# bellaj09/SGC

Hardware: AMD Instinct MI355X
Metric: propagated edges/sec (K-hop SpMM) + precompute wall-time, Reddit K=2 at 1/2/4/8 GPUs (higher is better)
Workload: dtype f32; 1 GPU; reddit-shape sgc_precompute K=2; nodes=232965, undirected_edges=11606919, nnz=23446803, features=602, hops=2, parallelism=single-gpu

## Files before the change

### include/sgc_amd.h

```cpp
#ifndef SGC_AMD_H
#define SGC_AMD_H

#include <stddef.h>
#include <stdint.h>

#ifdef __cplusplus
extern "C" {
#endif

#define SGC_ABI_VERSION 1

enum {
    SGC_OK = 0,
    SGC_EINVAL = 1,
    SGC_ERANGE = 2,
    SGC_EHIP = 3,
    SGC_ENOMEM = 4,
    SGC_EDEVICE = 5
};

int sgc_abi_version(void);
const char *sgc_last_error(void);

int sgc_set_tuning(const char *key, int64_t value);
// ... 238 lines not shown
                         const float *X, int64_t ldx, float *Y, int64_t ldy, int64_t F,
                         int32_t n_threads);
int sgc_spmm_csr_f32_cpu_ex(const int32_t *row_ptr, const int32_t *col_idx, const float *val,
                            int64_t row_begin, int64_t row_end,
                            const float *X, int64_t ldx, float *Y, int64_t ldy, int64_t F,
                            uint32_t flags, int32_t n_threads);
int64_t sgc_propagate_cpu_workspace(int64_t n_rows, int64_t F, int32_t K);
int sgc_propagate_f32_cpu(const int32_t *row_ptr, const int32_t *col_idx, const float *val,
                          int64_t n_rows, const float *X0, int64_t ldx, float *out,
                          int64_t ldo, int64_t F, int32_t K, void *workspace,
                          int64_t workspace_bytes, int32_t n_threads);

int64_t sgc_plan_sorted_workspace(int64_t n_rows);
int sgc_plan_sorted(const int32_t *row_ptr, int64_t row_begin, int64_t row_end,
                    int32_t threshold, int32_t hub_threshold, int32_t *plan, void *workspace,
                    int64_t workspace_bytes, int64_t *counts_host, void *stream);
int sgc_plan_sorted_ex(const int32_t *row_ptr, int64_t row_begin, int64_t row_end,
                       int32_t threshold, int32_t hub_threshold, int32_t *plan, void *workspace,
                       int64_t workspace_bytes, int64_t *counts_host, void *stream);
int sgc_plan_sorted_ex2(const int32_t *row_ptr, int64_t row_begin, int64_t row_end,
                        int32_t threshold, int32_t hub_threshold, int32_t *plan, void *workspace,
                        int64_t workspace_bytes, int64_t *counts_host, void *stream);

int64_t sgc_colsplit_workspace(int64_t n_rows, int32_t groups);
int sgc_csr_colsplit(const int32_t *row_ptr, const int32_t *col_idx, const float *val,
                     int64_t n_rows, int64_t n_cols, int32_t groups, const int32_t *cuts_host,
                     int32_t *row_ptrs, int32_t *col_out, float *val_out, void *workspace,
                     int64_t workspace_bytes, void *stream);
int sgc_csr_colsplit_ex(const int32_t *row_ptr, const int32_t *col_idx, const float *val,
                        int64_t n_rows, int64_t n_cols, int32_t groups,
                        const int32_t *cuts_host, int32_t whole_rows, int32_t *row_ptrs,
                        int32_t *col_out, float *val_out, void *workspace,
                        int64_t workspace_bytes, void *stream);

int sgc_mgpu_init(int ndev, const int *devices);
int sgc_mgpu_attach(const int32_t *row_ptr, const int32_t *col_idx, const float *val,
                    int64_t n_rows, int64_t nnz, void *stream, int64_t *handle);
int sgc_mgpu_propagate(int64_t handle, const float *X0, int64_t ldx, float *out, int64_t ldo,
                       int64_t F, int32_t K, void *stream);
int sgc_mgpu_detach(int64_t handle);
int sgc_mgpu_finalize(void);

enum { SGC_WARM_PROPAGATE = 1, SGC_WARM_CLASSIFIER = 2, SGC_WARM_LOADERS = 4 };
int sgc_warmup(uint32_t units, void *stream);

#ifdef __cplusplus
}
#endif
#endif
```

### sgc_amd/_lib.py

```python
import ctypes
import os

import torch

_HERE = os.path.dirname(os.path.abspath(__file__))
LIB_PATH = os.environ.get("SGC_AMD_LIB", os.path.join(_HERE, "libsgc_amd.so"))

_i64, _i32, _u32 = ctypes.c_int64, ctypes.c_int32, ctypes.c_uint32
_p, _sz = ctypes.c_void_p, ctypes.c_size_t

SIGNATURES = {
    "sgc_abi_version": (ctypes.c_int, []),
    "sgc_last_error": (ctypes.c_char_p, []),
    "sgc_set_tuning": (ctypes.c_int, [ctypes.c_char_p, _i64]),
    "sgc_get_tuning": (_i64, [ctypes.c_char_p]),
    "sgc_coo_to_csr_workspace": (ctypes.c_int, [_i64, _i64, ctypes.POINTER(_sz)]),
    "sgc_coo_to_csr": (ctypes.c_int, [_p, _p, _p, _i64, _i64, _i64, _p, _p, _p, _p, _sz,
                                      ctypes.POINTER(_u32), _p]),
    "sgc_csr64_to_csr": (ctypes.c_int, [_p, _p, _p, _i64, _i64, _i64, _p, _p, _p,
                                        ctypes.POINTER(_u32), _p]),
    "sgc_augnorm_workspace": (_i64, [_i64]),
    "sgc_augnorm_count": (ctypes.c_int, [_p, _p, _p, _i64, _i64, _p, _p, _p, _i64,
                                         ctypes.POINTER(_i64), ctypes.POINTER(_u32), _p]),
    "sgc_augnorm_fill": (ctypes.c_int, [_p, _p, _p, _i64, _p, _p, _p, _p, _p, _i64,
# ... 47 lines not shown
                                                    _i64, _i32, _i32, _i32]),
    "sgc_launch_list_add_pad_rows": (ctypes.c_int, [_i64, _p, _i64, _p, _i64, _i64, _i64, _i32,
                                                    _i32]),
    "sgc_launch_list_run": (ctypes.c_int, [_i64, _p, _p, _p]),
    "sgc_launch_list_destroy": (ctypes.c_int, [_i64]),
    "sgc_linear_f32": (ctypes.c_int, [_p, _i64, _p, _p, _p, _i64, _i64, _i64, _i64, _p]),
    "sgc_linear_kernel_name": (ctypes.c_char_p, [_i64, _i64, _i64, _i64, _p]),
    "sgc_linear_backward_kernel_name": (ctypes.c_char_p, [_i64, _i64, _i64, _i64, _p]),
    "sgc_cross_entropy_workspace": (_i64, [_i64, _i64]),
    "sgc_cross_entropy_f32": (ctypes.c_int, [_p, _i64, _p, _i64, _i64, _i64, _p, _p, _p, _p, _i64,
                                             _p]),
    "sgc_cross_entropy_backward_f32": (ctypes.c_int, [_p, _i64, _p, _p, _p, _p, _i64, _i64, _i64,
                                                      _p, _i64, _p]),
    "sgc_linear_xent_workspace": (_i64, [_i64, _i64, _i64]),
    "sgc_linear_xent_f32": (ctypes.c_int, [_p, _i64, _p, _p, _p, _i64, _i64, _i64, _p, _p, _p,
                                           _p, _i64, _p, _i64, _p]),
    "sgc_timing_enable": (ctypes.c_int, [ctypes.c_int]),
    "sgc_timing_collect": (ctypes.c_int, [_p, _p, _i64, ctypes.POINTER(_i64)]),
    "sgc_timing_collect_ex": (ctypes.c_int, [_p, _p, _p, _p, _i64, ctypes.POINTER(_i64)]),
    "sgc_coo_to_csr_cpu": (ctypes.c_int, [_p, _p, _p, _i64, _i64, _i64, _p, _p, _p,
                                          ctypes.POINTER(_u32)]),
    "sgc_spmm_csr_f32_cpu": (ctypes.c_int, [_p, _p, _p, _i64, _i64, _p, _i64, _p, _i64, _i64,
                                            _i32]),
    "sgc_spmm_csr_f32_cpu_ex": (ctypes.c_int, [_p, _p, _p, _i64, _i64, _p, _i64, _p, _i64, _i64,
                                               ctypes.c_uint32, _i32]),
    "sgc_propagate_cpu_workspace": (_i64, [_i64, _i64, _i32]),
    "sgc_propagate_f32_cpu": (ctypes.c_int, [_p, _p, _p, _i64, _p, _i64, _p, _i64, _i64, _i32,
                                             _p, _i64, _i32]),
    "sgc_colsplit_workspace": (_i64, [_i64, _i32]),
    "sgc_csr_colsplit": (ctypes.c_int, [_p, _p, _p, _i64, _i64, _i32, _p, _p, _p, _p, _p, _i64,
                                        _p]),
    "sgc_csr_colsplit_ex": (ctypes.c_int, [_p, _p, _p, _i64, _i64, _i32, _p, _i32, _p, _p, _p, _p,
                                           _i64, _p]),
    "sgc_plan_sorted_workspace": (_i64, [_i64]),
    "sgc_plan_sorted": (ctypes.c_int, [_p, _i64, _i64, _i32, _i32, _p, _p, _i64, _p, _p]),
    "sgc_plan_sorted_ex": (ctypes.c_int, [_p, _i64, _i64, _i32, _i32, _p, _p, _i64, _p, _p]),
    "sgc_plan_sorted_ex2": (ctypes.c_int, [_p, _i64, _i64, _i32, _i32, _p, _p, _i64, _p, _p]),
    "sgc_mgpu_init": (ctypes.c_int, [ctypes.c_int, _p]),
    "sgc_mgpu_attach": (ctypes.c_int, [_p, _p, _p, _i64, _i64, _p, ctypes.POINTER(_i64)]),
    "sgc_mgpu_propagate": (ctypes.c_int, [_i64, _p, _i64, _p, _i64, _i64, _i32, _p]),
    "sgc_mgpu_detach": (ctypes.c_int, [_i64]),
    "sgc_mgpu_finalize": (ctypes.c_int, []),
    "sgc_warmup": (ctypes.c_int, [_u32, _p]),
    "sgc_linear_backward_workspace": (_i64, [_i64, _i64, _i64]),
    "sgc_linear_backward_f32": (ctypes.c_int, [_p, _i64, _p, _i64, _i64, _i64, _i64, _p, _p, _p,
                                               _i64, _p]),
    "sgc_linear_x16": (ctypes.c_int, [_p, _i32, _i64, _p, _p, _p, _i64, _i64, _i64, _i64, _p]),
    "sgc_linear_x16_kernel_name": (ctypes.c_char_p, [_i64, _i64, _i64, _i64, _p, _i32]),
    "sgc_linear_backward_x16_workspace": (_i64, [_i64, _i64, _i64]),
    "sgc_linear_backward_x16": (ctypes.c_int, [_p, _i32, _i64, _p, _i64, _i64, _i64, _i64, _p, _p,
                                               _p, _i64, _p]),
    "sgc_linear_backward_x16_kernel_name": (ctypes.c_char_p, [_i64, _i64, _i64, _i64, _p, _i32]),
    "sgc_lbfgs_workspace": (_i64, [_i64, _i32]),
    "sgc_lbfgs_init": (ctypes.c_int, [_p, _i64, _i64, _i32, _p]),
    "sgc_lbfgs_begin_step": (ctypes.c_int, [_p, _p]),
    "sgc_lbfgs_iterate_f32": (ctypes.c_int, [_p, _i32, _p, _p, _p, _p, ctypes.c_double, _i32, _i32,
                                             ctypes.c_double, ctypes.c_double, _p]),
    "sgc_lbfgs_read_status": (ctypes.c_int, [_p, ctypes.POINTER(_i64), _p]),
    "sgc_adam_step_f32": (ctypes.c_int, [_i32, _p, _p, _p, _p, _p, _i64, ctypes.c_double,
                                         ctypes.c_double, ctypes.c_double, ctypes.c_double,
                                         ctypes.c_double, _p]),
    "sgc_train_adam_workspace": (_i64, [_i64, _i64, _i64]),
    "sgc_train_adam_f32": (ctypes.c_int, [_p, _i64, _p, _p, _p, _i64, _i64, _i64, _p, _p, _p, _p,
                                          _i64, _i32, ctypes.c_double, ctypes.c_double,
                                          ctypes.c_double, ctypes.c_double, ctypes.c_double, _p,
                                          _p, _i64, _p]),
# ... 46 lines not shown
```

### sgc_amd/csrc/capi.hip

```cpp
#include <cstdarg>
#include <map>
#include <mutex>
#include <vector>
#include <cstdio>
#include <cstring>

#include "common.h"

namespace sgc {

static thread_local char g_err[512] = "";

void set_error(const char *fmt, ...) {
    va_list ap;
    va_start(ap, fmt);
    vsnprintf(g_err, sizeof(g_err), fmt, ap);
    va_end(ap);
}

int coo_to_csr_workspace(int64_t n_rows, int64_t nnz, size_t *bytes);
int coo_to_csr(const int64_t *rows, const int64_t *cols, const float *vals, int64_t nnz,
               int64_t n_rows, int64_t n_cols, int32_t *row_ptr, int32_t *col_idx,
               float *val_out, void *ws, size_t ws_bytes, uint32_t *status_host,
               hipStream_t stream);
// ... 79 lines not shown
const char *linear_backward_kernel_name(int64_t M, int64_t K, int64_t ldx, int64_t C,
                                        const float *X);
int launch_linear_f32(const float *X, int64_t ldx, const float *W, const float *b, float *Y,
                      int64_t ldy, int64_t M, int64_t K, int64_t C, hipStream_t stream);
const char *linear_x16_kernel_name(int64_t M, int64_t K, int64_t ldx, int64_t C, const void *X,
                                   int32_t x_dtype);
int launch_linear_x16(const void *X, int32_t x_dtype, int64_t ldx, const float *W, const float *b,
                      float *Y, int64_t ldy, int64_t M, int64_t K, int64_t C, hipStream_t stream);
const char *linear_backward_x16_kernel_name(int64_t M, int64_t K, int64_t ldx, int64_t C,
                                            const void *X, int32_t x_dtype);
int64_t linear_backward_x16_workspace_bytes(int64_t M, int64_t K, int64_t C);
int linear_backward_x16(const void *X, int32_t x_dtype, int64_t ldx, const float *dY, int64_t ldd,
                        int64_t M, int64_t K, int64_t C, float *dW, float *db, void *ws,
                        int64_t ws_bytes, hipStream_t s);
int64_t plan_sorted_workspace(int64_t n_rows);
int plan_sorted(const int32_t *row_ptr, int64_t row_begin, int64_t row_end, int32_t threshold,
                int32_t hub_threshold, int32_t *plan, void *workspace, int64_t workspace_bytes,
                int64_t *counts_host, hipStream_t stream);
int plan_sorted_ex(const int32_t *row_ptr, int64_t row_begin, int64_t row_end, int32_t threshold,
                   int32_t hub_threshold, int32_t *plan, void *workspace,
                   int64_t workspace_bytes, int64_t *counts_host, hipStream_t stream);
int plan_sorted_ex2(const int32_t *row_ptr, int64_t row_begin, int64_t row_end, int32_t threshold,
                    int32_t hub_threshold, int32_t *plan, void *workspace,
                    int64_t workspace_bytes, int64_t *counts_host, hipStream_t stream);
int64_t colsplit_workspace(int64_t n_rows, int32_t groups);
int colsplit(const int32_t *row_ptr, const int32_t *col_idx, const float *val, int64_t n_rows,
             int64_t n_cols, int32_t groups, const int32_t *cuts_host, int32_t *row_ptrs,
             int32_t *col_out, float *val_out, void *workspace, int64_t workspace_bytes,
             hipStream_t stream);
int colsplit_ex(const int32_t *row_ptr, const int32_t *col_idx, const float *val, int64_t n_rows,
                int64_t n_cols, int32_t groups, const int32_t *cuts_host, int32_t whole_rows,
                int32_t *row_ptrs, int32_t *col_out, float *val_out, void *workspace,
                int64_t workspace_bytes, hipStream_t stream);
int mgpu_init(int ndev, const int *devices);
int mgpu_finalize();
int mgpu_attach(const int32_t *row_ptr, const int32_t *col_idx, const float *val, int64_t n,
                int64_t nnz, hipStream_t stream, int64_t *handle);
int mgpu_detach(int64_t handle);
int mgpu_propagate(int64_t handle, const float *X, int64_t ldx, float *Y, int64_t ldy, int64_t F,
                   int32_t K, hipStream_t stream);
int64_t lbfgs_workspace(int64_t n, int32_t history_size);
int lbfgs_init(void *state, int64_t bytes, int64_t n, int32_t history_size, hipStream_t s);
int lbfgs_begin_step(void *state, hipStream_t s);
int lbfgs_iterate(void *state, int32_t n_tensors, float *const *params, const float *const *grads,
                  const int64_t *numels, const float *loss, double lr, int32_t max_iter,
                  int32_t max_eval, double tol_grad, double tol_change, hipStream_t s);
int lbfgs_read_status(const void *state, int64_t *out_host, hipStream_t s);
extern int g_adam_kernel, g_adam_kernel_last;
int adam_set_tuning(int64_t value);
int64_t adam_small_max_rows();
int adam_step(int32_t n_tensors, float *const *params, const float *const *grads,
              float *const *exp_avgs, float *const *exp_avg_sqs, const int64_t *numels,
              int64_t step, double lr, double beta1, double beta2, double eps, double weight_decay,
              hipStream_t s);
int64_t train_adam_workspace(int64_t M, int64_t K, int64_t C);
int train_adam(const float *X, int64_t ldx, float *W, float *b, const int64_t *labels, int64_t M,
               int64_t K, int64_t C, float *mW, float *vW, float *mb, float *vb, int64_t step0,
               int32_t epochs, double lr, double beta1, double beta2, double eps,
               double weight_decay, float *loss_trace, void *ws, int64_t ws_bytes, hipStream_t s);
hipError_t warm_adam(hipStream_t);

}

using namespace sgc;

extern "C" {
// ... 694 lines not shown
                    int64_t n_rows, int64_t nnz, void *stream, int64_t *handle) {
    return mgpu_attach(row_ptr, col_idx, val, n_rows, nnz, as_stream(stream), handle);
}

int sgc_mgpu_propagate(int64_t handle, const float *X0, int64_t ldx, float *out, int64_t ldo,
                       int64_t F, int32_t K, void *stream) {
    return mgpu_propagate(handle, X0, ldx, out, ldo, F, K, as_stream(stream));
}

int sgc_mgpu_detach(int64_t handle) { return mgpu_detach(handle); }

int sgc_mgpu_finalize(void) { return mgpu_finalize(); }

int64_t sgc_colsplit_workspace(int64_t n_rows, int32_t groups) {
    return colsplit_workspace(n_rows, groups);
}

int sgc_csr_colsplit(const int32_t *row_ptr, const int32_t *col_idx, const float *val,
                     int64_t n_rows, int64_t n_cols, int32_t groups, const int32_t *cuts_host,
                     int32_t *row_ptrs, int32_t *col_out, float *val_out, void *workspace,
                     int64_t workspace_bytes, void *stream) {
    return colsplit(row_ptr, col_idx, val, n_rows, n_cols, groups, cuts_host, row_ptrs, col_out,
                    val_out, workspace, workspace_bytes, as_stream(stream));
}

int sgc_csr_colsplit_ex(const int32_t *row_ptr, const int32_t *col_idx, const float *val,
                        int64_t n_rows, int64_t n_cols, int32_t groups, const int32_t *cuts_host,
                        int32_t whole_rows, int32_t *row_ptrs, int32_t *col_out, float *val_out,
                        void *workspace, int64_t workspace_bytes, void *stream) {
    return colsplit_ex(row_ptr, col_idx, val, n_rows, n_cols, groups, cuts_host, whole_rows,
                       row_ptrs, col_out, val_out, workspace, workspace_bytes, as_stream(stream));
}

int64_t sgc_plan_sorted_workspace(int64_t n_rows) { return plan_sorted_workspace(n_rows); }

int sgc_plan_sorted(const int32_t *row_ptr, int64_t row_begin, int64_t row_end,
                    int32_t threshold, int32_t hub_threshold, int32_t *plan, void *workspace,
                    int64_t workspace_bytes, int64_t *counts_host, void *stream) {
    return plan_sorted(row_ptr, row_begin, row_end, threshold, hub_threshold, plan, workspace,
                       workspace_bytes, counts_host, as_stream(stream));
}

int sgc_plan_sorted_ex2(const int32_t *row_ptr, int64_t row_begin, int64_t row_end,
                        int32_t threshold, int32_t hub_threshold, int32_t *plan, void *workspace,
                        int64_t workspace_bytes, int64_t *counts_host, void *stream) {
    return plan_sorted_ex2(row_ptr, row_begin, row_end, threshold, hub_threshold, plan, workspace,
                           workspace_bytes, counts_host, as_stream(stream));
}

int sgc_plan_sorted_ex(const int32_t *row_ptr, int64_t row_begin, int64_t row_end,
                       int32_t threshold, int32_t hub_threshold, int32_t *plan, void *workspace,
                       int64_t workspace_bytes, int64_t *counts_host, void *stream) {
    return plan_sorted_ex(row_ptr, row_begin, row_end, threshold, hub_threshold, plan, workspace,
                          workspace_bytes, counts_host, as_stream(stream));
}
```

### sgc_amd/csrc/groups.hip

```cpp
#include "common.h"

#include <algorithm>
#include <cstdlib>

namespace sgc {

namespace {

constexpr int kGroupsMax = 8;
constexpr int kThreads = 256;

struct Cuts {
    int32_t c[kGroupsMax + 1];
};

__device__ __forceinline__ int32_t lower_bound(const int32_t *__restrict__ col, int32_t lo,
                                               int32_t hi, int32_t v) {
    while (lo < hi) {
        const int32_t mid = lo + ((hi - lo) >> 1);
        if (col[mid] < v) lo = mid + 1;
        else hi = mid;
    }
    return lo;
}

__global__ void colsplit_count_kernel(const int32_t *__restrict__ row_ptr,
                                      const int32_t *__restrict__ col, int32_t n, int32_t chunk,
                                      int G, Cuts cuts, int32_t whole_rows,
                                      int32_t *__restrict__ counts,
                                      int32_t *__restrict__ block_sums) {
    __shared__ int32_t s_sum[kGroupsMax];
    if (threadIdx.x < kGroupsMax) s_sum[threadIdx.x] = 0;
    __syncthreads();
    const int32_t r0 = blockIdx.x * chunk, r1 = min(n, r0 + chunk);
    int32_t mine[kGroupsMax] = {0, 0, 0, 0, 0, 0, 0, 0};
    for (int32_t r = r0 + threadIdx.x; r < r1; r += blockDim.x) {
        const int32_t k0 = row_ptr[r], k1 = row_ptr[r + 1];
        const bool whole = k1 - k0 <= whole_rows;
        int32_t lo = k0;
        for (int g = 0; g < G; ++g) {
            const int32_t hi =
                (whole || g + 1 == G) ? k1 : lower_bound(col, lo, k1, cuts.c[g + 1]);
            counts[(int64_t)g * n + r] = hi - lo;
            mine[g] += hi - lo;
            lo = hi;
        }
    }
    for (int g = 0; g < G; ++g)
        if (mine[g]) atomicAdd(&s_sum[g], mine[g]);
    __syncthreads();
    if (threadIdx.x < G) block_sums[threadIdx.x * gridDim.x + blockIdx.x] = s_sum[threadIdx.x];
}

__global__ void colsplit_scan_blocks_kernel(int32_t *__restrict__ block_sums, int nblk, int G) {
    if (threadIdx.x != 0 || blockIdx.x != 0) return;
    int32_t run = 0;
    for (int g = 0; g < G; ++g)
        for (int b = 0; b < nblk; ++b) {
            const int32_t v = block_sums[g * nblk + b];
            block_sums[g * nblk + b] = run;
            run += v;
        }
}

__global__ void colsplit_rowptr_kernel(const int32_t *__restrict__ counts, int32_t n,
                                       int32_t chunk, int G,
                                       const int32_t *__restrict__ block_off,
                                       int32_t *__restrict__ row_ptrs) {
    __shared__ int32_t s[kThreads];
    __shared__ int32_t s_carry;
    const int32_t r0 = blockIdx.x * chunk, r1 = min(n, r0 + chunk);
    for (int g = 0; g < G; ++g) {
        const int32_t *cnt = counts + (int64_t)g * n;
        int32_t *rp = row_ptrs + (int64_t)g * (n + 1);
        if (threadIdx.x == 0) s_carry = block_off[g * gridDim.x + blockIdx.x];
        __syncthreads();
        for (int32_t base = r0; base < r1; base += kThreads) {
            const int32_t r = base + threadIdx.x;
            const int32_t v = r < r1 ? cnt[r] : 0;
            s[threadIdx.x] = v;
            __syncthreads();
            for (int o = 1; o < kThreads; o <<= 1) {
                const int32_t add = threadIdx.x >= o ? s[threadIdx.x - o] : 0;
                __syncthreads();
                s[threadIdx.x] += add;
                __syncthreads();
            }
            const int32_t carry = s_carry;
            if (r < r1) rp[r] = carry + s[threadIdx.x] - v;
            __syncthreads();
            if (threadIdx.x == kThreads - 1) s_carry = carry + s[kThreads - 1];
            __syncthreads();
        }
        if (r1 == n && r0 < r1 && threadIdx.x == 0) rp[n] = s_carry;
        __syncthreads();
    }
}

__global__ void colsplit_fill_kernel(const int32_t *__restrict__ row_ptr,
                                     const int32_t *__restrict__ col,
                                     const float *__restrict__ val, int32_t n, int G, Cuts cuts,
                                     int32_t whole_rows, const int32_t *__restrict__ row_ptrs,
                                     int32_t *__restrict__ col_out, float *__restrict__ val_out) {
    const int lane = threadIdx.x & (kWave - 1);
    const int64_t waves = (int64_t)gridDim.x * (blockDim.x / kWave);
    for (int64_t r = (int64_t)blockIdx.x * (blockDim.x / kWave) + threadIdx.x / kWave; r < n;
         r += waves) {
        const int32_t k0 = row_ptr[r], k1 = row_ptr[r + 1];
        if (k1 - k0 <= whole_rows) {
            const int32_t dst = row_ptrs[r];
            for (int32_t k = k0 + lane; k < k1; k += kWave) {
                col_out[dst + (k - k0)] = col[k];
                val_out[dst + (k - k0)] = val[k];
            }
            continue;
        }
        int32_t lo = k0;
        for (int g = 0; g < G; ++g) {
            const int32_t hi = (g + 1 == G) ? k1 : lower_bound(col, lo, k1, cuts.c[g + 1]);
            const int32_t dst = row_ptrs[(int64_t)g * (n + 1) + r];
            for (int32_t k = lo + lane; k < hi; k += kWave) {
                col_out[dst + (k - lo)] = col[k];
                val_out[dst + (k - lo)] = val[k];
            }
            lo = hi;
        }
    }
}

constexpr size_t kAlign = 256;
size_t up(size_t b) { return (b + kAlign - 1) / kAlign * kAlign; }

int nblocks(int64_t n) { return (int)std::max<int64_t>(1, std::min<int64_t>(1024, (n + 1023) / 1024)); }

}

int64_t colsplit_workspace(int64_t n_rows, int32_t groups) {
    if (n_rows <= 0 || groups <= 0) return (int64_t)kAlign;
    return (int64_t)(up((size_t)groups * n_rows * sizeof(int32_t)) +
                     up((size_t)groups * nblocks(n_rows) * sizeof(int32_t)));
}

int colsplit_ex(const int32_t *row_ptr, const int32_t *col_idx, const float *val, int64_t n_rows,
                int64_t n_cols, int32_t groups, const int32_t *cuts_host, int32_t whole_rows,
                int32_t *row_ptrs, int32_t *col_out, float *val_out, void *workspace,
                int64_t workspace_bytes, hipStream_t stream) {
    SGC_REQUIRE(whole_rows >= 0, SGC_EINVAL, "colsplit: whole_rows must be >= 0");
    SGC_REQUIRE(groups >= 1 && groups <= kGroupsMax, SGC_EINVAL,
                "colsplit: groups must be 1..%d", kGroupsMax);
    SGC_REQUIRE(n_rows >= 0 && n_rows < INT32_MAX && n_cols >= 0 && n_cols < INT32_MAX,
                SGC_ERANGE, "colsplit: bad shape");
    SGC_REQUIRE(row_ptr && row_ptrs && cuts_host && workspace, SGC_EINVAL,
                "colsplit: null pointer");
    SGC_REQUIRE(cuts_host[0] == 0 && cuts_host[groups] == n_cols, SGC_EINVAL,
                "colsplit: cuts must run from 0 to n_cols");
    Cuts cuts{};
    for (int g = 0; g <= groups; ++g) {
        SGC_REQUIRE(g == 0 || cuts_host[g] >= cuts_host[g - 1], SGC_EINVAL,
                    "colsplit: cuts must not decrease");
        cuts.c[g] = cuts_host[g];
    }
    if (n_rows == 0) {
        for (int g = 0; g < groups; ++g)
            SGC_HIP_CHECK(hipMemsetAsync(row_ptrs + g, 0, sizeof(int32_t), stream));
        return SGC_OK;
    }
    SGC_REQUIRE(workspace_bytes >= colsplit_workspace(n_rows, groups), SGC_ENOMEM,
                "colsplit: workspace %lld < %lld bytes", (long long)workspace_bytes,
                (long long)colsplit_workspace(n_rows, groups));
    SGC_REQUIRE(col_out && val_out, SGC_EINVAL, "colsplit: null output");
    const int32_t n = (int32_t)n_rows;
    const int nblk = nblocks(n_rows);
    const int32_t chunk = (int32_t)((n_rows + nblk - 1) / nblk);
    char *w = static_cast<char *>(workspace);
    int32_t *counts = reinterpret_cast<int32_t *>(w);
    w += up((size_t)groups * n_rows * sizeof(int32_t));
    int32_t *block_sums = reinterpret_cast<int32_t *>(w);
    hipLaunchKernelGGL(colsplit_count_kernel, dim3(nblk), dim3(kThreads), 0, stream, row_ptr,
                       col_idx, n, chunk, (int)groups, cuts, whole_rows, counts, block_sums);
    SGC_HIP_CHECK(hipGetLastError());
    hipLaunchKernelGGL(colsplit_scan_blocks_kernel, dim3(1), dim3(kWave), 0, stream, block_sums,
                       nblk, (int)groups);
    SGC_HIP_CHECK(hipGetLastError());
    hipLaunchKernelGGL(colsplit_rowptr_kernel, dim3(nblk), dim3(kThreads), 0, stream, counts, n,
                       chunk, (int)groups, block_sums, row_ptrs);
    SGC_HIP_CHECK(hipGetLastError());
    const int fill_blocks = (int)std::min<int64_t>((n_rows + 3) / 4, 8192);
    hipLaunchKernelGGL(colsplit_fill_kernel, dim3(fill_blocks), dim3(kThreads), 0, stream, row_ptr,
                       col_idx, val, n, (int)groups, cuts, whole_rows, row_ptrs, col_out, val_out);
    SGC_HIP_CHECK(hipGetLastError());
    return SGC_OK;
}

int colsplit(const int32_t *row_ptr, const int32_t *col_idx, const float *val, int64_t n_rows,
             int64_t n_cols, int32_t groups, const int32_t *cuts_host, int32_t *row_ptrs,
             int32_t *col_out, float *val_out, void *workspace, int64_t workspace_bytes,
             hipStream_t stream) {
    return colsplit_ex(row_ptr, col_idx, val, n_rows, n_cols, groups, cuts_host, 0, row_ptrs,
                       col_out, val_out, workspace, workspace_bytes, stream);
}

__global__ void cols_ascending_kernel(const int32_t *__restrict__ row_ptr,
                                      const int32_t *__restrict__ col, int64_t n,
                                      int32_t *__restrict__ bad) {
    for (int64_t i = blockIdx.x * (int64_t)blockDim.x + threadIdx.x; i < n;
         i += (int64_t)gridDim.x * blockDim.x) {
        for (int32_t k = row_ptr[i] + 1; k < row_ptr[i + 1]; ++k)
            if (col[k - 1] >= col[k]) {
                atomicOr(bad, 1);
                break;
            }
    }
}

int csr_cols_ascending(const int32_t *row_ptr, const int32_t *col_idx, int64_t n_rows,
                       hipStream_t stream, bool *ascending) {
    SGC_REQUIRE(row_ptr && ascending, SGC_EINVAL, "cols_ascending: null pointer");
    *ascending = true;
    if (n_rows <= 0) return SGC_OK;
    int32_t *bad = nullptr;
    SGC_HIP_CHECK(hipMallocAsync((void **)&bad, sizeof(int32_t), stream));
    SGC_HIP_CHECK(hipMemsetAsync(bad, 0, sizeof(int32_t), stream));
    const int blocks = (int)std::min<int64_t>((n_rows + 255) / 256, 4096);
    hipLaunchKernelGGL(cols_ascending_kernel, dim3(blocks), dim3(256), 0, stream, row_ptr,
// ... 27 lines not shown
```

### sgc_amd/propagate.py

```python
import os
from dataclasses import dataclass, field
from typing import NamedTuple, Optional

import numpy as np
import torch

from . import _lib

_HEAVY_ENV = os.environ.get("SGC_AMD_HEAVY_THRESHOLD")
DEFAULT_HEAVY_THRESHOLD = int(_HEAVY_ENV) if _HEAVY_ENV else None
_HUB_ENV = os.environ.get("SGC_AMD_HUB_THRESHOLD")
DEFAULT_HUB_THRESHOLD = int(_HUB_ENV) if _HUB_ENV else None
HUB_SHARE = 1024
HUB_CAP, HUB_CAP_BELOW_NNZ = 8192, 1 << 24


def auto_heavy_threshold(nnz_range, width):
    import math
    work = max(1.0, int(nnz_range) * max(1, int(width)) / float(1 << 23))
    return int(min(512, max(64, 1 << int(round(math.log2(work))))))


def auto_hub_threshold(nnz_range, heavy_threshold):
    hub = int(nnz_range) // HUB_SHARE
# ... 47 lines not shown
            csr._plans[key] = int(((rp[1:] - rp[:-1]) > ts).sum().item())
        above = csr._plans[key]
    return max(0, above - pl.n_heavy), int(ts)

SLOT_FIXED, SLOT_X0, SLOT_OUT = 0, 1, 2
SPMM_X_PADDED = 1
SPMM_Y_PADDED = 2
SPMM_NO_HUB = 4
SPMM_HUB_ONLY = 8
SPMM_ACCUMULATE = 16
SPMM_HUB_SERIAL = 32
SPMM_LIGHT_ORDER = 64
SPMM_X_UNDER_4G = 128


def x_flags(X):
    n, ld = X.shape[0], X.stride(0)
    return SPMM_X_UNDER_4G if n < (1 << 24) and n * ld * 4 < (1 << 32) else 0
LIGHT_ORDER = os.environ.get("SGC_AMD_LIGHT_ORDER", "1") != "0"
HUB_SERIAL_MAX_DEGREE = 3072

STATUS_ROWS_SORTED = 1
STATUS_COLS_ASCENDING = 2
STATUS_OUT_OF_RANGE = 4

_GROUPS_ENV = os.environ.get("SGC_AMD_COLUMN_GROUPS")
COLUMN_GROUPS = int(_GROUPS_ENV) if _GROUPS_ENV else None
GROUPS_MIN_NNZ = 1 << 22
GROUPS_MIN_WIDTH = 128
GROUPS_WIDE_NNZ = 1 << 26
_WHOLE_ENV = os.environ.get("SGC_AMD_GROUP_WHOLE_ROWS")
GROUP_WHOLE_ROWS = int(_WHOLE_ENV) if _WHOLE_ENV else None
GROUP_WHOLE_ROWS_RULE = 32


def group_whole_rows_for(csr, G):
    if G <= 1:
        return 0
    if GROUP_WHOLE_ROWS is not None:
        return max(0, int(GROUP_WHOLE_ROWS))
    return GROUP_WHOLE_ROWS_RULE


def column_groups_for(csr, width):
    if csr.device.type != "cuda" or not csr.cols_ascending or csr.nnz == 0:
        return 1
    if COLUMN_GROUPS is not None:
        return max(1, min(8, int(COLUMN_GROUPS), max(1, csr.n_cols)))
    if width < GROUPS_MIN_WIDTH or csr.nnz < GROUPS_MIN_NNZ:
        return 1
    if csr.nnz >= GROUPS_WIDE_NNZ:
        return 4
    if 128 < width <= 256:
        return 1
    return 2


def _host_cols_ascending(row_ptr, col_idx):
    if isinstance(row_ptr, torch.Tensor):
        if row_ptr.device.type != "cpu" or col_idx.device.type != "cpu":
            return False
        row_ptr, col_idx = row_ptr.numpy(), col_idx.numpy()
    rp = np.asarray(row_ptr, dtype=np.int64)
    ci = np.asarray(col_idx)
    if ci.size < 2:
        return True
    bad = np.diff(ci.astype(np.int64)) <= 0
    starts = rp[1:-1]
    starts = starts[(starts > 0) & (starts < ci.size)]
    bad[starts - 1] = False
    return not bool(bad.any())


def _require_device(t, what):
    if not isinstance(t, torch.Tensor):
        raise TypeError(f"sgc_amd: {what} must be a torch.Tensor")
    if t.device.type != "cuda":
        raise RuntimeError(
            f"sgc_amd: {what} is on {t.device}; the propagation engine runs only on a "
            "ROCm (gfx950) device -- move tensors with .cuda() (no CPU fallback)")


def cpu_threads():
    return max(1, torch.get_num_threads())


@dataclass
class DeviceCSR:
    n_rows: int
    n_cols: int
    row_ptr: torch.Tensor
    col_idx: torch.Tensor
    val: torch.Tensor
    status: int = 0
    ingest_seconds: float = 0.0
    _plans: dict = field(default_factory=dict)

    @property
    def nnz(self):
        return self.col_idx.numel()

    @property
    def device(self):
        return self.row_ptr.device

    @property
    def cols_ascending(self):
        return bool(self.status & STATUS_COLS_ASCENDING)

    def group_cuts(self, G):
        return [(g * self.n_cols) // G for g in range(G + 1)]

    def column_groups(self, G, whole_rows=0):
        if not self.cols_ascending:
            raise ValueError("sgc_amd: column groups need rows with ascending columns")
        whole_rows = int(whole_rows)
        if whole_rows < 0:
            raise ValueError("sgc_amd: whole_rows must be >= 0")
        whole_rows = min(whole_rows, 2 ** 31 - 1)
        key = ("groups", int(G), whole_rows)
        if key not in self._plans:
            import ctypes
            lib = _lib.load()
            n, nnz, dev = self.n_rows, self.nnz, self.device
            cuts = (ctypes.c_int32 * (G + 1))(*self.group_cuts(G))
            row_ptrs = torch.empty((G, n + 1), dtype=torch.int32, device=dev)
            col = torch.empty(max(1, nnz), dtype=torch.int32, device=dev)
            val = torch.empty(max(1, nnz), dtype=torch.float32, device=dev)
            ws_bytes = lib.sgc_colsplit_workspace(n, G)
            ws = torch.empty(max(1, ws_bytes), dtype=torch.uint8, device=dev)
            with torch.cuda.device(dev):
                _lib.check(lib.sgc_csr_colsplit_ex(_lib.ptr(self.row_ptr), _lib.ptr(self.col_idx),
                                                   _lib.ptr(self.val), n, self.n_cols, G,
                                                   ctypes.cast(cuts, ctypes.c_void_p), whole_rows,
                                                   _lib.ptr(row_ptrs), _lib.ptr(col),
                                                   _lib.ptr(val), _lib.ptr(ws), ws_bytes,
                                                   _lib.stream_handle(dev)), "csr_colsplit")
            del ws
            self._plans[key] = [DeviceCSR(n, self.n_cols, row_ptrs[g], col[:nnz], val[:nnz],
                                          self.status) for g in range(G)]
        return self._plans[key]

    def release_prepared(self):
        for key in [k for k in self._plans if isinstance(k, tuple) and k[:1] == ("list",)]:
            del self._plans[key]

    def drop_groups(self):
        self.release_prepared()
        for key in [k for k in self._plans if isinstance(k, tuple) and k[:1] == ("groups",)]:
            for part in self._plans.pop(key):
                part._plans.clear()

    def groups_or_self(self, G):
        if G <= 1:
            return [self]
        try:
            return self.column_groups(G, group_whole_rows_for(self, G))
        except torch.cuda.OutOfMemoryError:
            return [self]

    @classmethod
    def from_host_arrays(cls, row_ptr, col_idx, val, n_cols=None, device="cuda"):
        status = STATUS_COLS_ASCENDING if _host_cols_ascending(row_ptr, col_idx) else 0
        rp = torch.as_tensor(row_ptr).to(device=device, dtype=torch.int32)
        ci = torch.as_tensor(col_idx).to(device=device, dtype=torch.int32)
        va = torch.as_tensor(val).to(device=device, dtype=torch.float32)
        n = rp.numel() - 1
        return cls(n, n if n_cols is None else n_cols, rp.contiguous(), ci.contiguous(),
                   va.contiguous(), status)

    @classmethod
    def from_torch(cls, adj):
        import time
        if isinstance(adj, torch.Tensor) and adj.device.type == "cpu":
            return cls._from_torch_cpu(adj)
        _require_device(adj, "adj")
        if adj.dtype != torch.float32:
            raise TypeError(f"sgc_amd: adj must be float32, got {adj.dtype}")
        if adj.dim() != 2:
            raise ValueError("sgc_amd: adj must be 2-D")
        lib = _lib.load()
        n_rows, n_cols = adj.shape
        dev = adj.device
        t0 = time.perf_counter()
        with torch.cuda.device(dev):
            stream = _lib.stream_handle(dev)
            status = _lib._u32(0)
            if adj.layout == torch.sparse_coo:
                idx = adj._indices().contiguous()
                vals = adj._values().contiguous()
# ... 431 lines not shown
    n, F = X.shape
    if is_x16(X):
        if native_loop:
            require_f32_features(X, "propagate(native_loop=True)")
        if K <= 0:
            return X
        return _propagate_x16(csr, X, K, out, use_plan, threshold, hub_threshold, hop_hook,
                              out_dtype)
    if out_dtype not in (None, torch.float32):
        raise TypeError(f"sgc_amd: float32 features give float32 output, not {out_dtype}")
    if out is None:
        out = torch.empty((n, F), dtype=torch.float32, device=X.device)
    if n == 0 or F == 0 or K <= 0:
        if K <= 0:
            out.copy_(X)
        return out
    lib = _lib.load()
    if X.device.type == "cpu":
        ws_bytes = lib.sgc_propagate_cpu_workspace(n, F, int(K))
        ws = torch.empty(max(1, ws_bytes), dtype=torch.uint8)
        _lib.check(lib.sgc_propagate_f32_cpu(_lib.ptr(csr.row_ptr), _lib.ptr(csr.col_idx),
                                             _lib.ptr(csr.val), n, _lib.ptr(X), X.stride(0),
                                             _lib.ptr(out), out.stride(0), F, int(K), _lib.ptr(ws),
                                             ws_bytes, cpu_threads()), "propagate_f32_cpu")
        return out
    stream = torch.cuda.current_stream(X.device).cuda_stream
    G_rule = column_groups_for(csr, F) if use_plan else 1
    wide_knob, wide_ts = short_wide_state()
    key = None
    if (not native_loop and hop_hook is None and prepare and X.data_ptr() != out.data_ptr()
            and not torch.cuda.is_current_stream_capturing()):
        key = ("list", X.stride(0), F, int(K), out.stride(0), X.data_ptr() % 128 == 0,
               threshold, hub_threshold, bool(use_plan), G_rule,
               group_whole_rows_for(csr, G_rule), stream, PAD_X0, wide_knob, wide_ts)
        prep = csr._plans.get(key)
        if prep is not None:
            rc = lib.sgc_launch_list_run(prep[1].handle, X.data_ptr(), out.data_ptr(), stream)
            if rc:
                _lib.check(rc, "propagate (launch list)")
            return out
    groups = csr.groups_or_self(G_rule)
    G = len(groups)
    if G > 1:
        pl = None
        parts = [(c, c.plan(0, n, threshold, hub_threshold, F)) for c in groups]
    else:
        pl = csr.plan(0, n, threshold, hub_threshold, F) if use_plan else NO_PLAN
        parts = [(csr, pl)]
    parts = [(c, cp, cp.hub_flags() | (SPMM_ACCUMULATE if g else 0))
             for g, (c, cp) in enumerate(parts)]
    wide = [wide_args(c, cp, 0, n, wide_ts) for c, cp, _ in parts]
    ldw = aligned_ld(F)
    with torch.cuda.device(X.device):
        if native_loop:
            import ctypes
            Gn = len(parts)
            ws_bytes = lib.sgc_propagate_workspace(n, F, X.stride(0), K)
            ws = torch.empty(max(1, ws_bytes), dtype=torch.uint8, device=X.device)
            planned = use_plan and all(cp.rows is not None for _, cp, _ in parts)
            plans = (ctypes.c_void_p * Gn)(*[cp.rows.data_ptr() if planned else None
                                             for _, cp, _ in parts])
            n_heavy = (ctypes.c_int64 * Gn)(*[cp.n_heavy for _, cp, _ in parts])
            n_hub = (ctypes.c_int64 * Gn)(*[cp.n_hub for _, cp, _ in parts])
            ths = (ctypes.c_int32 * Gn)(*[cp.threshold for _, cp, _ in parts])
            pflags = (ctypes.c_uint32 * Gn)(*[cp.hub_flags() for _, cp, _ in parts])
            nonempty = (ctypes.c_int64 * Gn)(*[cp.n_nonempty for _, cp, _ in parts])
            not_wide = (ctypes.c_int64 * Gn)(*[w[0] for w in wide])
# ... 335 lines not shown
```

Before: 6.683 billion edges/s.

## Add coarse column-group ladder so medium rows split into fewer groups

Extends the column-split of the CSR with a second threshold. Rows up to whole_rows stay whole, rows up to coarse_rows are split into coarse_groups pieces, and only longer rows are split into all G groups. The default rule now raises G (for example 2 to 4, or 4 to 8) for large workloads and uses a coarse level for medium-degree rows. The aim is to keep column-blocked cache locality for long rows while cutting per-group row overhead and fragmentation for medium rows. The cost is more groups and more complex split logic, which can add per-group launches or imbalance.

```diff
diff --git a/include/sgc_amd.h b/include/sgc_amd.h
--- a/include/sgc_amd.h
+++ b/include/sgc_amd.h
@@ -294,6 +294,11 @@
                         const int32_t *cuts_host, int32_t whole_rows, int32_t *row_ptrs,
                         int32_t *col_out, float *val_out, void *workspace,
                         int64_t workspace_bytes, void *stream);
+int sgc_csr_colsplit_ex2(const int32_t *row_ptr, const int32_t *col_idx, const float *val,
+                         int64_t n_rows, int64_t n_cols, int32_t groups,
+                         const int32_t *cuts_host, int32_t whole_rows, int32_t coarse_rows,
+                         int32_t coarse_groups, int32_t *row_ptrs, int32_t *col_out,
+                         float *val_out, void *workspace, int64_t workspace_bytes, void *stream);
 
 int sgc_mgpu_init(int ndev, const int *devices);
 int sgc_mgpu_attach(const int32_t *row_ptr, const int32_t *col_idx, const float *val,
diff --git a/sgc_amd/_lib.py b/sgc_amd/_lib.py
--- a/sgc_amd/_lib.py
+++ b/sgc_amd/_lib.py
@@ -103,6 +103,8 @@
                                         _p]),
     "sgc_csr_colsplit_ex": (ctypes.c_int, [_p, _p, _p, _i64, _i64, _i32, _p, _i32, _p, _p, _p, _p,
                                            _i64, _p]),
+    "sgc_csr_colsplit_ex2": (ctypes.c_int, [_p, _p, _p, _i64, _i64, _i32, _p, _i32, _i32, _i32, _p,
+                                            _p, _p, _p, _i64, _p]),
     "sgc_plan_sorted_workspace": (_i64, [_i64]),
     "sgc_plan_sorted": (ctypes.c_int, [_p, _i64, _i64, _i32, _i32, _p, _p, _i64, _p, _p]),
     "sgc_plan_sorted_ex": (ctypes.c_int, [_p, _i64, _i64, _i32, _i32, _p, _p, _i64, _p, _p]),
diff --git a/sgc_amd/csrc/capi.hip b/sgc_amd/csrc/capi.hip
--- a/sgc_amd/csrc/capi.hip
+++ b/sgc_amd/csrc/capi.hip
@@ -135,6 +135,11 @@
                 int64_t n_cols, int32_t groups, const int32_t *cuts_host, int32_t whole_rows,
                 int32_t *row_ptrs, int32_t *col_out, float *val_out, void *workspace,
                 int64_t workspace_bytes, hipStream_t stream);
+int colsplit_ex2(const int32_t *row_ptr, const int32_t *col_idx, const float *val,
+                 int64_t n_rows, int64_t n_cols, int32_t groups, const int32_t *cuts_host,
+                 int32_t whole_rows, int32_t coarse_rows, int32_t coarse_groups,
+                 int32_t *row_ptrs, int32_t *col_out, float *val_out, void *workspace,
+                 int64_t workspace_bytes, hipStream_t stream);
 int mgpu_init(int ndev, const int *devices);
 int mgpu_finalize();
 int mgpu_attach(const int32_t *row_ptr, const int32_t *col_idx, const float *val, int64_t n,
@@ -895,6 +900,16 @@
                        row_ptrs, col_out, val_out, workspace, workspace_bytes, as_stream(stream));
 }
 
+int sgc_csr_colsplit_ex2(const int32_t *row_ptr, const int32_t *col_idx, const float *val,
+                         int64_t n_rows, int64_t n_cols, int32_t groups,
+                         const int32_t *cuts_host, int32_t whole_rows, int32_t coarse_rows,
+                         int32_t coarse_groups, int32_t *row_ptrs, int32_t *col_out,
+                         float *val_out, void *workspace, int64_t workspace_bytes, void *stream) {
+    return colsplit_ex2(row_ptr, col_idx, val, n_rows, n_cols, groups, cuts_host, whole_rows,
+                        coarse_rows, coarse_groups, row_ptrs, col_out, val_out, workspace,
+                        workspace_bytes, as_stream(stream));
+}
+
 int64_t sgc_plan_sorted_workspace(int64_t n_rows) { return plan_sorted_workspace(n_rows); }
 
 int sgc_plan_sorted(const int32_t *row_ptr, int64_t row_begin, int64_t row_end,
diff --git a/sgc_amd/csrc/groups.hip b/sgc_amd/csrc/groups.hip
--- a/sgc_amd/csrc/groups.hip
+++ b/sgc_amd/csrc/groups.hip
@@ -24,9 +24,15 @@
     return lo;
 }
 
+__device__ __forceinline__ int row_step(int32_t len, int G, int32_t whole_rows,
+                                        int32_t coarse_rows, int coarse_step) {
+    return len <= whole_rows ? G : len <= coarse_rows ? coarse_step : 1;
+}
+
 __global__ void colsplit_count_kernel(const int32_t *__restrict__ row_ptr,
                                       const int32_t *__restrict__ col, int32_t n, int32_t chunk,
                                       int G, Cuts cuts, int32_t whole_rows,
+                                      int32_t coarse_rows, int coarse_step,
                                       int32_t *__restrict__ counts,
                                       int32_t *__restrict__ block_sums) {
     __shared__ int32_t s_sum[kGroupsMax];
@@ -36,11 +42,12 @@
     int32_t mine[kGroupsMax] = {0, 0, 0, 0, 0, 0, 0, 0};
     for (int32_t r = r0 + threadIdx.x; r < r1; r += blockDim.x) {
         const int32_t k0 = row_ptr[r], k1 = row_ptr[r + 1];
-        const bool whole = k1 - k0 <= whole_rows;
+        const int step = row_step(k1 - k0, G, whole_rows, coarse_rows, coarse_step);
         int32_t lo = k0;
         for (int g = 0; g < G; ++g) {
-            const int32_t hi =
-                (whole || g + 1 == G) ? k1 : lower_bound(col, lo, k1, cuts.c[g + 1]);
+            int32_t hi = lo;
+            if (g % step == 0)
+                hi = g + step >= G ? k1 : lower_bound(col, lo, k1, cuts.c[g + step]);
             counts[(int64_t)g * n + r] = hi - lo;
             mine[g] += hi - lo;
             lo = hi;
@@ -100,7 +107,8 @@
 __global__ void colsplit_fill_kernel(const int32_t *__restrict__ row_ptr,
                                      const int32_t *__restrict__ col,
                                      const float *__restrict__ val, int32_t n, int G, Cuts cuts,
-                                     int32_t whole_rows, const int32_t *__restrict__ row_ptrs,
+                                     int32_t whole_rows, int32_t coarse_rows, int coarse_step,
+                                     const int32_t *__restrict__ row_ptrs,
                                      int32_t *__restrict__ col_out, float *__restrict__ val_out) {
     const int lane = threadIdx.x & (kWave - 1);
     const int64_t waves = (int64_t)gridDim.x * (blockDim.x / kWave);
@@ -115,9 +123,10 @@
             }
             continue;
         }
+        const int step = row_step(k1 - k0, G, whole_rows, coarse_rows, coarse_step);
         int32_t lo = k0;
-        for (int g = 0; g < G; ++g) {
-            const int32_t hi = (g + 1 == G) ? k1 : lower_bound(col, lo, k1, cuts.c[g + 1]);
+        for (int g = 0; g < G; g += step) {
+            const int32_t hi = g + step >= G ? k1 : lower_bound(col, lo, k1, cuts.c[g + step]);
             const int32_t dst = row_ptrs[(int64_t)g * (n + 1) + r];
             for (int32_t k = lo + lane; k < hi; k += kWave) {
                 col_out[dst + (k - lo)] = col[k];
@@ -141,13 +150,18 @@
                      up((size_t)groups * nblocks(n_rows) * sizeof(int32_t)));
 }
 
-int colsplit_ex(const int32_t *row_ptr, const int32_t *col_idx, const float *val, int64_t n_rows,
-                int64_t n_cols, int32_t groups, const int32_t *cuts_host, int32_t whole_rows,
-                int32_t *row_ptrs, int32_t *col_out, float *val_out, void *workspace,
-                int64_t workspace_bytes, hipStream_t stream) {
+int colsplit_ex2(const int32_t *row_ptr, const int32_t *col_idx, const float *val,
+                 int64_t n_rows, int64_t n_cols, int32_t groups, const int32_t *cuts_host,
+                 int32_t whole_rows, int32_t coarse_rows, int32_t coarse_groups,
+                 int32_t *row_ptrs, int32_t *col_out, float *val_out, void *workspace,
+                 int64_t workspace_bytes, hipStream_t stream) {
     SGC_REQUIRE(whole_rows >= 0, SGC_EINVAL, "colsplit: whole_rows must be >= 0");
     SGC_REQUIRE(groups >= 1 && groups <= kGroupsMax, SGC_EINVAL,
                 "colsplit: groups must be 1..%d", kGroupsMax);
+    SGC_REQUIRE(coarse_groups >= 1 && groups % coarse_groups == 0, SGC_EINVAL,
+                "colsplit: coarse_groups %d must divide groups %d", coarse_groups, groups);
+    SGC_REQUIRE(coarse_rows >= whole_rows, SGC_EINVAL,
+                "colsplit: coarse_rows %d < whole_rows %d", coarse_rows, whole_rows);
     SGC_REQUIRE(n_rows >= 0 && n_rows < INT32_MAX && n_cols >= 0 && n_cols < INT32_MAX,
                 SGC_ERANGE, "colsplit: bad shape");
     SGC_REQUIRE(row_ptr && row_ptrs && cuts_host && workspace, SGC_EINVAL,
@@ -170,6 +184,7 @@
                 (long long)colsplit_workspace(n_rows, groups));
     SGC_REQUIRE(col_out && val_out, SGC_EINVAL, "colsplit: null output");
     const int32_t n = (int32_t)n_rows;
+    const int coarse_step = (int)(groups / coarse_groups);
     const int nblk = nblocks(n_rows);
     const int32_t chunk = (int32_t)((n_rows + nblk - 1) / nblk);
     char *w = static_cast<char *>(workspace);
@@ -177,7 +192,8 @@
     w += up((size_t)groups * n_rows * sizeof(int32_t));
     int32_t *block_sums = reinterpret_cast<int32_t *>(w);
     hipLaunchKernelGGL(colsplit_count_kernel, dim3(nblk), dim3(kThreads), 0, stream, row_ptr,
-                       col_idx, n, chunk, (int)groups, cuts, whole_rows, counts, block_sums);
+                       col_idx, n, chunk, (int)groups, cuts, whole_rows, coarse_rows, coarse_step,
+                       counts, block_sums);
     SGC_HIP_CHECK(hipGetLastError());
     hipLaunchKernelGGL(colsplit_scan_blocks_kernel, dim3(1), dim3(kWave), 0, stream, block_sums,
                        nblk, (int)groups);
@@ -187,9 +203,19 @@
     SGC_HIP_CHECK(hipGetLastError());
     const int fill_blocks = (int)std::min<int64_t>((n_rows + 3) / 4, 8192);
     hipLaunchKernelGGL(colsplit_fill_kernel, dim3(fill_blocks), dim3(kThreads), 0, stream, row_ptr,
-                       col_idx, val, n, (int)groups, cuts, whole_rows, row_ptrs, col_out, val_out);
+                       col_idx, val, n, (int)groups, cuts, whole_rows, coarse_rows, coarse_step, row_ptrs,
+                       col_out, val_out);
     SGC_HIP_CHECK(hipGetLastError());
     return SGC_OK;
+}
+
+int colsplit_ex(const int32_t *row_ptr, const int32_t *col_idx, const float *val, int64_t n_rows,
+                int64_t n_cols, int32_t groups, const int32_t *cuts_host, int32_t whole_rows,
+                int32_t *row_ptrs, int32_t *col_out, float *val_out, void *workspace,
+                int64_t workspace_bytes, hipStream_t stream) {
+    return colsplit_ex2(row_ptr, col_idx, val, n_rows, n_cols, groups, cuts_host, whole_rows,
+                        whole_rows, groups, row_ptrs, col_out, val_out, workspace,
+                        workspace_bytes, stream);
 }
 
 int colsplit(const int32_t *row_ptr, const int32_t *col_idx, const float *val, int64_t n_rows,
diff --git a/sgc_amd/propagate.py b/sgc_amd/propagate.py
--- a/sgc_amd/propagate.py
+++ b/sgc_amd/propagate.py
@@ -103,6 +103,13 @@
 _WHOLE_ENV = os.environ.get("SGC_AMD_GROUP_WHOLE_ROWS")
 GROUP_WHOLE_ROWS = int(_WHOLE_ENV) if _WHOLE_ENV else None
 GROUP_WHOLE_ROWS_RULE = 32
+_COARSE_GROUPS_ENV = os.environ.get("SGC_AMD_GROUP_COARSE_GROUPS")
+GROUP_COARSE_GROUPS = int(_COARSE_GROUPS_ENV) if _COARSE_GROUPS_ENV else None
+_COARSE_ROWS_ENV = os.environ.get("SGC_AMD_GROUP_COARSE_ROWS")
+GROUP_COARSE_ROWS = int(_COARSE_ROWS_ENV) if _COARSE_ROWS_ENV else None
+GROUP_COARSE_ROWS_RULE = 512
+GROUP_LADDER_RULE = {2: (4, 64), 4: (8, 512)}
+GROUP_LADDER_MIN_WORK = 11 << 30
 
 
 def group_whole_rows_for(csr, G):
@@ -113,11 +120,7 @@
     return GROUP_WHOLE_ROWS_RULE
 
 
-def column_groups_for(csr, width):
-    if csr.device.type != "cuda" or not csr.cols_ascending or csr.nnz == 0:
-        return 1
-    if COLUMN_GROUPS is not None:
-        return max(1, min(8, int(COLUMN_GROUPS), max(1, csr.n_cols)))
+def _size_rule_groups(csr, width):
     if width < GROUPS_MIN_WIDTH or csr.nnz < GROUPS_MIN_NNZ:
         return 1
     if csr.nnz >= GROUPS_WIDE_NNZ:
@@ -125,6 +128,40 @@
     if 128 < width <= 256:
         return 1
     return 2
+
+
+def group_coarse_for(csr, G):
+    T = group_whole_rows_for(csr, G)
+    if G <= 1:
+        return 1, 0
+    Gc, H = G, GROUP_COARSE_ROWS_RULE
+    if COLUMN_GROUPS is None:
+        coarse = 4 if csr.nnz >= GROUPS_WIDE_NNZ else 2
+        fine, rows = GROUP_LADDER_RULE.get(coarse, (coarse, H))
+        if fine == G:
+            Gc, H = coarse, rows
+    if GROUP_COARSE_GROUPS is not None and G % max(1, int(GROUP_COARSE_GROUPS)) == 0:
+        Gc = max(1, int(GROUP_COARSE_GROUPS))
+    if GROUP_COARSE_ROWS is not None:
+        H = int(GROUP_COARSE_ROWS)
+    return (Gc, max(H, T)) if Gc != G else (G, T)
+
+
+def group_ladder_for(csr, width):
+    if csr.device.type != "cuda" or not csr.cols_ascending or csr.nnz == 0:
+        return 1, 1, 0
+    if COLUMN_GROUPS is not None:
+        G = max(1, min(8, int(COLUMN_GROUPS), max(1, csr.n_cols)))
+    else:
+        G = _size_rule_groups(csr, width)
+        measured = {4: 128 < width <= 256, 2: csr.nnz * width >= GROUP_LADDER_MIN_WORK}
+        if measured.get(G):
+            G = GROUP_LADDER_RULE.get(G, (G,))[0]
+    return (G, *group_coarse_for(csr, G))
+
+
+def column_groups_for(csr, width):
+    return group_ladder_for(csr, width)[0]
 
 
 def _host_cols_ascending(row_ptr, col_idx):
@@ -182,14 +219,25 @@
     def group_cuts(self, G):
         return [(g * self.n_cols) // G for g in range(G + 1)]
 
-    def column_groups(self, G, whole_rows=0):
+    def column_groups(self, G, whole_rows=0, coarse_rows=None, coarse_groups=None):
         if not self.cols_ascending:
             raise ValueError("sgc_amd: column groups need rows with ascending columns")
         whole_rows = int(whole_rows)
         if whole_rows < 0:
             raise ValueError("sgc_amd: whole_rows must be >= 0")
         whole_rows = min(whole_rows, 2 ** 31 - 1)
-        key = ("groups", int(G), whole_rows)
+        G = int(G)
+        coarse_groups = G if coarse_groups is None else int(coarse_groups)
+        if coarse_groups < 1 or G % coarse_groups:
+            raise ValueError(f"sgc_amd: coarse_groups {coarse_groups} must divide G = {G}")
+        if coarse_groups == G or coarse_rows is None:
+            coarse_groups, coarse_rows = G, whole_rows
+        coarse_rows = min(int(coarse_rows), 2 ** 31 - 1)
+        if coarse_rows < whole_rows:
+            raise ValueError("sgc_amd: coarse_rows must be >= whole_rows")
+        key = ("groups", G, whole_rows)
+        if coarse_groups != G:
+            key += (coarse_rows, coarse_groups)
         if key not in self._plans:
             import ctypes
             lib = _lib.load()
@@ -201,12 +249,14 @@
             ws_bytes = lib.sgc_colsplit_workspace(n, G)
             ws = torch.empty(max(1, ws_bytes), dtype=torch.uint8, device=dev)
             with torch.cuda.device(dev):
-                _lib.check(lib.sgc_csr_colsplit_ex(_lib.ptr(self.row_ptr), _lib.ptr(self.col_idx),
-                                                   _lib.ptr(self.val), n, self.n_cols, G,
-                                                   ctypes.cast(cuts, ctypes.c_void_p), whole_rows,
-                                                   _lib.ptr(row_ptrs), _lib.ptr(col),
-                                                   _lib.ptr(val), _lib.ptr(ws), ws_bytes,
-                                                   _lib.stream_handle(dev)), "csr_colsplit")
+                _lib.check(lib.sgc_csr_colsplit_ex2(_lib.ptr(self.row_ptr),
+                                                    _lib.ptr(self.col_idx), _lib.ptr(self.val), n,
+                                                    self.n_cols, G,
+                                                    ctypes.cast(cuts, ctypes.c_void_p), whole_rows,
+                                                    coarse_rows, coarse_groups,
+                                                    _lib.ptr(row_ptrs), _lib.ptr(col),
+                                                    _lib.ptr(val), _lib.ptr(ws), ws_bytes,
+                                                    _lib.stream_handle(dev)), "csr_colsplit")
             del ws
             self._plans[key] = [DeviceCSR(n, self.n_cols, row_ptrs[g], col[:nnz], val[:nnz],
                                           self.status) for g in range(G)]
@@ -226,7 +276,8 @@
         if G <= 1:
             return [self]
         try:
-            return self.column_groups(G, group_whole_rows_for(self, G))
+            Gc, H = group_coarse_for(self, G)
+            return self.column_groups(G, group_whole_rows_for(self, G), H, Gc)
         except torch.cuda.OutOfMemoryError:
             return [self]
 
@@ -724,7 +775,8 @@
             and not torch.cuda.is_current_stream_capturing()):
         key = ("list", X.stride(0), F, int(K), out.stride(0), X.data_ptr() % 128 == 0,
                threshold, hub_threshold, bool(use_plan), G_rule,
-               group_whole_rows_for(csr, G_rule), stream, PAD_X0, wide_knob, wide_ts)
+               group_whole_rows_for(csr, G_rule), group_coarse_for(csr, G_rule), stream, PAD_X0,
+               wide_knob, wide_ts)
         prep = csr._plans.get(key)
         if prep is not None:
             rc = lib.sgc_launch_list_run(prep[1].handle, X.data_ptr(), out.data_ptr(), stream)
```

After: 6.823 billion edges/s, median of 6. +2.1%, better.
